# apirrone/Open_Duck_Playground

Measured on AMD Instinct MI355X. Metric: env-steps/sec open_duck_mini_v2 flat_terrain @8192 envs; 1/2/4/8-GPU scaling, higher is better.
Workload: dtype f32

## Files before the change

### open_duck_playground_amd/csrc/odk_engine.hip

```cpp
#include <hip/hip_runtime.h>
#include <stddef.h>

#include <cmath>
#include <cstdarg>
#include <cstdio>
#include <cstdlib>
#include <cstring>
#include <array>
#include <string>
#include <vector>

#include "../../include/odk.h"
#include "odk_kernels.h"

using namespace odk;

struct RecLay {
  int CMD, LAST, LAST2, LAST3, MT, AIR, PEAK, PUSH, AHIST, IMU, EPSTEPS, TRUNC, DONE, EPSUM, EPLEN, EPMET, KEY0, KEY1, CTR, STEP, PSTEP, PINT, IMI, LCON, NINFO;
};
constexpr RecLay rec_lay(int nu) {
  RecLay r{};
  r.CMD = 0; r.LAST = 7; r.LAST2 = r.LAST + nu; r.LAST3 = r.LAST2 + nu; r.MT = r.LAST3 + nu; r.AIR = r.MT + nu; r.PEAK = r.AIR + 2; r.PUSH = r.PEAK + 2;
  r.AHIST = r.PUSH + 2; r.IMU = r.AHIST + 3 * nu; r.EPSTEPS = r.IMU + 9; r.TRUNC = r.EPSTEPS + 1; r.DONE = r.TRUNC + 1; r.EPSUM = r.DONE + 1; r.EPLEN = r.EPSUM + 1;
  r.EPMET = r.EPLEN + 1; r.KEY0 = r.EPMET + ODK_NMETRIC; r.KEY1 = r.KEY0 + 1; r.CTR = r.KEY1 + 1; r.STEP = r.CTR + 1; r.PSTEP = r.STEP + 1; r.PINT = r.PSTEP + 1;
// ... 206 lines not shown

__device__ inline void sample_command(const EnvCfg& c, uint32_t k0, uint32_t k1, uint32_t ctr, uint32_t base, int k, float& out) {
  const float z = rng_uniform(k0, k1, ctr, base + 7);
  const float u = rng_uniform(k0, k1, ctr, base + k);
  out = (z < 0.1f) ? 0.0f : c.cmd_range[k][0] + u * (c.cmd_range[k][1] - c.cmd_range[k][0]);
}

template <int NDRAW>
__device__ __forceinline__ void draw_block(uint32_t k0, uint32_t k1, uint32_t ctr, float* NZ, int lane) {
  uint32_t a, b;
  threefry2x32(k0, k1, ctr, (uint32_t)(lane + 2), a, b);
  if (lane < NDRAW / 2) { NZ[2 * lane] = (float)(a >> 8) * (1.0f / 16777216.0f); NZ[2 * lane + 1] = (float)(b >> 8) * (1.0f / 16777216.0f); }
  ODK_SYNC();
}

template <class S, int G, int KIND>
__device__ __forceinline__ void build_obs_kind(float* L, const DevModel* m, const EnvCfg& c, const float* contact, const float* NZ,
                          int imitation_i, const float* phase, int lane) {
  using E = EnvL<S>;
  float* P = L + E::O_PRIV; float* INFO = L + E::O_INFO; const float* SENS = L + S::O_SENS; const float* SCR = L + S::O_SCR;
  const float* QPOS = L + S::O_QPOS; const float* QVEL = L + S::O_QVEL;
  const float lvl = c.noise_level;
  constexpr int NU = S::NU;
  constexpr RecLay RL = rec_lay(NU);
  constexpr int NOBS = obs_nobs(NU, false), DQV = draw_qvel(NU) - 4;
  const float con0 = contact[0], con1 = contact[1], ph0 = phase[0], ph1 = phase[1];
  const int adr_gyro = m->adr_gyro, adr_acc = m->adr_accelerometer, adr_lin = m->adr_local_linvel, adr_ang = m->adr_global_angvel;
  float ng = 0;
  if (lane < 3) ng = SCR[S::S_MISC + 10 + lane] + (2.0f * NZ[10 - 4 + lane] - 1.0f) * lvl * c.noise_gravity;
  float h0 = 0, h1 = 0;
  if (lane < 3) { h0 = INFO[RL.IMU + lane]; h1 = INFO[RL.IMU + 3 + lane]; }
  ODK_SYNC();
  if (lane < 3) { INFO[RL.IMU + lane] = ng; INFO[RL.IMU + 3 + lane] = h0; INFO[RL.IMU + 6 + lane] = h1; }
  constexpr bool standing = KIND != 0;
  constexpr int NP = obs_npriv(NU, standing);
#pragma unroll
  for (int it = 0; it < (NP + G - 1) / G; it++) {
    const int ks = lane + it * G;
    __builtin_assume(ks >= it * G && ks < it * G + G);
    if (ks >= NP) continue;
    const int k = !standing ? ks : (ks < 13 + 5 * NU ? ks : (ks < 15 + 5 * NU ? ks + NU : ks + NOBS - (15 + 5 * NU)));
    const int q = k - NOBS;
    const int uA = min(max(k - 13, 0), NU - 1), uV = min(max(k - 13 - NU, 0), NU - 1), uQ = min(max(q - 15, 0), NU - 1), uQV = min(max(q - 15 - NU, 0), NU - 1);
    const int tF = min(max(q - 18 - 3 * NU, 0), 5);
    const int A_bq = m->act_backlash_qposadr[uA], A_aq = m->act_qposadr[uA], V_ad = m->act_dofadr[uV];
    const float A_kc = m->key_ctrl[uA], A_ns = c.qpos_noise_scale[uA];
    const int Q_bq = m->act_backlash_qposadr[uQ], Q_aq = m->act_qposadr[uQ], QV_ad = m->act_dofadr[uQV], F_adr = m->adr_foot_linvel[tF >= 3 ? 1 : 0];
    const float Q_kc = m->key_ctrl[uQ];
    {
      const int k_lo = standing ? 0 : it * G, k_hi = standing ? NP + NOBS : it * G + G;
      auto hits = [&](int lo, int hi) { return k_lo < hi && k_hi > lo; };
      if (hits(13, 13 + NU)) asm volatile("" :: "v"(A_bq), "v"(A_aq), "v"(A_kc), "v"(A_ns));
      if (hits(13 + NU, 13 + 2 * NU)) asm volatile("" :: "v"(V_ad));
      if (hits(NOBS + 15, NOBS + 15 + NU)) asm volatile("" :: "v"(Q_bq), "v"(Q_aq), "v"(Q_kc));
      if (hits(NOBS + 15 + NU, NOBS + 15 + 2 * NU)) asm volatile("" :: "v"(QV_ad));
      if (hits(NOBS + 18 + 3 * NU, NOBS + 24 + 3 * NU)) asm volatile("" :: "v"(F_adr));
    }
    float v = 0;
    if (k < 3) v = SENS[adr_gyro + k] + (2.0f * NZ[k] - 1.0f) * lvl * c.noise_gyro;
    else if (k < 6) v = SENS[adr_acc + k - 3] + (2.0f * NZ[k] - 1.0f) * lvl * c.noise_accelerometer;
    else if (k < 13) v = INFO[RL.CMD + k - 6];
    else if (k < 13 + NU) {
      const int u = k - 13;
      const float ja = QPOS[A_aq] + (A_bq >= 0 ? QPOS[A_bq] : 0.0f);
      v = ja + (2.0f * NZ[13 - 4 + u] - 1.0f) * lvl * A_ns - A_kc;
    } else if (k < 13 + 2 * NU) {
      const int u = k - 13 - NU;
      v = (QVEL[V_ad] + (2.0f * NZ[DQV + u] - 1.0f) * lvl * c.noise_joint_vel) * c.dof_vel_scale;
    } else if (k < 13 + 3 * NU) v = INFO[RL.LAST + k - 13 - 2 * NU];
    else if (k < 13 + 4 * NU) v = INFO[RL.LAST2 + k - 13 - 3 * NU];
    else if (k < 13 + 5 * NU) v = INFO[RL.LAST3 + k - 13 - 4 * NU];
    else if (k < 13 + 6 * NU) v = INFO[RL.MT + k - 13 - 5 * NU];
    else if (k < 15 + 6 * NU) v = (k - 13 - 6 * NU) ? con1 : con0;
    else if (k < 17 + 6 * NU) v = (k - 15 - 6 * NU) ? ph1 : ph0;
    else {
      if (q < 3) v = SENS[adr_gyro + q];
      else if (q < 6) v = SENS[adr_acc + q - 3];
      else if (q < 9) v = SCR[S::S_MISC + 10 + q - 6];
      else if (q < 12) v = SENS[adr_lin + q - 9];
      else if (q < 15) v = SENS[adr_ang + q - 12];
      else if (q < 15 + NU) v = QPOS[Q_aq] + (Q_bq >= 0 ? QPOS[Q_bq] : 0.0f) - Q_kc;
      else if (q < 15 + 2 * NU) v = QVEL[QV_ad];
      else if (q == 15 + 2 * NU) v = QPOS[2];
      else if (q < 16 + 3 * NU) v = L[S::O_ACTF + q - 16 - 2 * NU];
      else if (q < 18 + 3 * NU) v = (q - 16 - 3 * NU) ? con1 : con0;
      else if (q < 24 + 3 * NU) { const int t = q - 18 - 3 * NU; v = SENS[F_adr + (t >= 3 ? t - 3 : t)]; }
      else if (q < 26 + 3 * NU) v = INFO[RL.AIR + q - 24 - 3 * NU];
      else if (q < 66 + 3 * NU) v = L[E::O_REF + q - 26 - 3 * NU];
      else if (q == 66 + 3 * NU) v = (float)imitation_i;
      else v = (q - 67 - 3 * NU) ? ph1 : ph0;
    }
    P[ks] = v;
  }
  ODK_SYNC();
}
template <class S, int G>
__device__ __forceinline__ void build_obs(float* L, const DevModel* m, const EnvCfg& c, const float* contact, const float* NZ,
                          int imitation_i, const float* phase, int lane) {
  if (c.kind == 0) build_obs_kind<S, G, 0>(L, m, c, contact, NZ, imitation_i, phase, lane);
  else build_obs_kind<S, G, 1>(L, m, c, contact, NZ, imitation_i, phase, lane);
}

__device__ __forceinline__ void foot_contact_flags(const float* CDIST, float* contact) {
  for (int f = 0; f < 2; f++) {
    float md = 1e4f;
    for (int k = 0; k < 4; k++) md = fminf(md, CDIST[4 * f + k]);
    contact[f] = md < 0 ? 1.0f : 0.0f;
  }
}

template <class S, int G>
__device__ __forceinline__ void write_outputs(const KArgs& a, const float* L, int env, float reward, float done, float trunc, const float* metrics, int lane) {
  using E = EnvL<S>;
  const float* P = L + E::O_PRIV;
  const int nobs = a.cfg.nobs, npriv = a.cfg.npriv;
// ... 121 lines not shown
    if (a.cmd) v = a.cmd[(size_t)e * a.cmd_stride + lane];
    INFO[RL.CMD + lane] = v;
  }
  ODK_SYNC();
  forward_env<S, G, HF>(L, RT, m, a.hfield, st, lane, 1);
  if (a.dbg_lds && live) dump_lds<S, G>(a.dbg_lds, L, env, lane);
  const float pint = c.push_interval_range[0] + rng_uniform(k0, kr, 0, 17 + NU) * (c.push_interval_range[1] - c.push_interval_range[0]);
  const int push_interval_steps = (int)rintf(pint / c.ctrl_dt);
  if (c.use_imitation) prm_eval<G>(&a.prm, a.prm_table, INFO[RL.CMD], INFO[RL.CMD + 1], INFO[RL.CMD + 2], 0, L + E::O_REF, lane);
  else for (int k = lane; k < 40; k += G) L[E::O_REF + k] = 0;
  ODK_SYNC();
  float contact[2];
  foot_contact_flags(L + S::O_CDIST, contact);
  const float phase[2] = {0, 0};
  draw_block<E::NDRAW>(k0, k1, 0u, L + E::O_NZ, lane);
  build_obs<S, G>(L, m, c, contact, L + E::O_NZ, 0, phase, lane);
  if (lane == 0) {
    INFO[RL.KEY0] = i2f((int)k0); INFO[RL.KEY1] = i2f((int)k1); INFO[RL.CTR] = i2f(1);
    INFO[RL.STEP] = i2f(0); INFO[RL.PSTEP] = i2f(0); INFO[RL.PINT] = i2f(push_interval_steps);
    INFO[RL.IMI] = i2f(0); INFO[RL.LCON] = i2f(0);
  }
  ODK_SYNC();
  if (live) {
    float* rc = a.recs + (size_t)env * R::SIZE;
    float* fs = a.first + (size_t)env * R::FSIZE;
    for (int i = lane; i < S::NQ; i += G) { rc[i] = L[S::O_QPOS + i]; fs[i] = L[S::O_QPOS + i]; }
    for (int i = lane; i < S::NV; i += G) {
      rc[S::NQ + i] = L[S::O_QVEL + i]; fs[S::NQ + i] = L[S::O_QVEL + i];
      rc[S::NQ + S::NV + i] = L[S::O_WARM + i]; fs[S::NQ + S::NV + i] = L[S::O_WARM + i];
    }
    for (int k = lane; k < R::NPRIV; k += G) {
      if (k < R::NOBS) fs[R::FOBS + k] = L[E::O_PRIV + k];
      fs[R::FOBS + R::NOBS + k] = L[E::O_PRIV + k];
    }
    for (int k = lane; k < RL.NINFO; k += G) rc[R::INFO + k] = INFO[k];
    float metrics[ODK_NMETRIC] = {0, 0, 0, 0, 0, 0, 0, 0};
    write_outputs<S, G>(a, L, env, 0.0f, 0.0f, 0.0f, metrics, lane);
    if (a.xmet && lane < ODK_NXTERM) a.xmet[(size_t)env * ODK_NXTERM + lane] = 0.0f;
  }
}

constexpr int STEP_WAVES = 2;
template <class S, int G, int HF>
__global__ void __launch_bounds__(64, STEP_WAVES) step_kernel(KArgs a) {
  extern __shared__ float lds[];
  using E = EnvL<S>; using R = Rec<S>;
  constexpr int NU = S::NU;
  constexpr RecLay RL = rec_lay(NU);
  const int slot = threadIdx.x / G, lane = threadIdx.x % G;
  const int env = blockIdx.x * (64 / G) + slot;
  const bool live = env < a.nenv;
  const int e = live ? env : a.nenv - 1;
  float* L = lds + slot * E::TOTAL;
#ifdef ODK_PROFILE
  const long long t_k0 = clock64();
#endif
  const int* RT = load_shared<S>(lds, 64 / G, a.m);
#ifdef ODK_POISON_LDS
  for (int k = lane; k < E::TOTAL; k += G) L[k] = __int_as_float(0x7fc00000);
// ... 83 lines not shown
  ODK_SYNC();
#ifdef ODK_PROFILE
  const long long t_k1 = clock64();
  if (lane == 0) L[S::O_SCR + S::S_PROF + 18] = (float)(t_k1 - t_k0);
#endif
  HotSt hot;
  if constexpr (HF == 0) load_hot<S, G>(hot, m, st, lane);
  for (int s = 0; s < a.n_substeps; s++) {
    const bool last = s == a.n_substeps - 1;
    size_t opaque0 = 0;
    asm volatile("" : "+s"(opaque0));
    const DevModel* ms = reinterpret_cast<const DevModel*>(reinterpret_cast<const char*>(m) + opaque0);
    int lane_s = lane;
    asm volatile("" : "+v"(lane_s));
    __builtin_assume(lane_s >= 0 && lane_s < 64);
    if constexpr (HF == 0) forward_env<S, G, HF, true>(L, RT, ms, a.hfield, st, lane_s, last ? 1 : 0, hot);
    else forward_env<S, G, HF>(L, RT, ms, a.hfield, st, lane_s, last ? 1 : 0);
    if (last && a.dbg_lds && live) dump_lds<S, G>(a.dbg_lds, L, env, lane);
    euler_env<S, G>(L, ms, st, lane_s);
  }
#ifdef ODK_PROFILE
  const long long t_k2 = clock64();
#endif
  size_t opaque1 = 0;
  asm volatile("" : "+s"(opaque1));
  const DevModel* mp = reinterpret_cast<const DevModel*>(reinterpret_cast<const char*>(m) + opaque1);
  const uint32_t k0e = (uint32_t)f2i(INFO[RL.KEY0]), k1e = (uint32_t)f2i(INFO[RL.KEY1]), ctre = (uint32_t)f2i(INFO[RL.CTR]);
  const int imi_e = f2i(INFO[RL.IMI]);
  const float phase_e[2] = {ACT[NU], ACT[NU + 1]};
  int step_e = f2i(INFO[RL.STEP]), push_step_e = f2i(INFO[RL.PSTEP]);
  float ep_steps_e = INFO[RL.EPSTEPS];
  const float prev_done_e = INFO[RL.DONE];
  for (int u = lane; u < NU; u += G) INFO[RL.MT + u] = CTRL[u];
  draw_block<E::NDRAW>(k0e, k1e, ctre, L + E::O_NZ, lane);
  if (lane < 40) L[E::O_REF + lane] = ref0;
  if (lane < 8) L[E::O_REF + 32 + lane] = ref1;
  ODK_SYNC();
  float contact[2];
  foot_contact_flags(L + S::O_CDIST, contact);
  float air[2], peak[2];
  for (int f = 0; f < 2; f++) {
    air[f] = INFO[RL.AIR + f] + dt;
    peak[f] = fmaxf(INFO[RL.PEAK + f], L[S::O_SCR + S::S_MISC + 8 + f]);
  }
  int fc_bits = 0;
  if (a.xt) {
    const int lc = f2i(INFO[RL.LCON]);
    for (int f = 0; f < 2; f++) fc_bits |= (INFO[RL.AIR + f] > 0.0f && (contact[f] != 0.0f || ((lc >> f) & 1))) ? 1 << f : 0;
  }
// ... 55 lines not shown
      const float lin_z = expf(-8.0f * (bv[2] - REF[36]) * (bv[2] - REF[36]));
      const float ang_xy = expf(-2.0f * ((bv[3] - REF[37]) * (bv[3] - REF[37]) + (bv[4] - REF[38]) * (bv[4] - REF[38]))) * 0.5f;
      const float ang_z = expf(-2.0f * (bv[5] - REF[39]) * (bv[5] - REF[39])) * 0.5f;
      float crew = 0;
      for (int f = 0; f < 2; f++) crew += (contact[f] == (REF[32 + f] > 0.5f ? 1.0f : 0.0f)) ? 1.0f : 0.0f;
      float r = lin_xy + lin_z + ang_xy + ang_z - t_jp * 15.0f - t_jv * 1.0e-3f + crew;
      r *= (cn > 0.01f) ? 1.0f : 0.0f;
      rew[6] = nan_to_num(r);
    }
  }
  float total = 0;
  for (int k = 0; k < 7; k++) { rew[k] *= c.reward_scales[k]; total += rew[k]; }
  if (a.xt) reward_library<S, G>(a, L, mp, contact, air, peak, fc_bits, done_env, total, env, live, lane);
  const float reward = fminf(fmaxf(total * dt, 0.0f), 10000.0f);
  const float* NZ = L + E::O_NZ;
  build_obs<S, G>(L, mp, c, contact, NZ, imi_e, phase_e, lane);
  step_e += 1; push_step_e += 1;
  float la = 0, lla = 0;
  for (int u = lane; u < NU; u += G) { la = INFO[RL.LAST + u]; lla = INFO[RL.LAST2 + u]; }
  ODK_SYNC();
  for (int u = lane; u < NU; u += G) { INFO[RL.LAST3 + u] = lla; INFO[RL.LAST2 + u] = la; INFO[RL.LAST + u] = ACT[u]; }
  if (step_e > 500 && lane < 7 && !a.cmd) {
    constexpr int DC = draw_cmd(NU) - 4;
    const float z = NZ[DC + 7], u = NZ[DC + lane];
    INFO[RL.CMD + lane] = (z < 0.1f) ? 0.0f : c.cmd_range[lane][0] + u * (c.cmd_range[lane][1] - c.cmd_range[lane][0]);
  }
  if (done_env || step_e > 500) step_e = 0;
  int lcon_new = 0;
  for (int f = 0; f < 2; f++) {
    if (contact[f] != 0.0f) { air[f] = 0; peak[f] = 0; lcon_new |= (1 << f); }
  }
// ... 21 lines not shown
    for (int k = lane; k < R::NPRIV; k += G) L[E::O_PRIV + k] = fs[R::FOBS + R::NOBS + k];
    if (a.cmd && lane >= 6 && lane < 13) L[E::O_PRIV + lane] = INFO[RL.CMD + lane - 6];
  }
  if (live) {
    int e_out = e;
    asm volatile("" : "+v"(e_out));
    float* rco = reinterpret_cast<float*>(reinterpret_cast<char*>(a.recs + (size_t)e_out * R::SIZE) + opaque1);
    for (int i = lane; i < S::NQ + 2 * S::NV; i += G) rco[i] = L[S::O_QPOS + i];
    for (int k = lane; k < RL.NINFO; k += G) rco[R::INFO + k] = INFO[k];
    write_outputs<S, G>(a, L, env, reward, done_f, trunc, metrics, lane);
  }
#ifdef ODK_PROFILE
  if (a.dbg_lds && live && lane == 0) a.dbg_lds[(size_t)env * S::TOTAL + S::O_SCR + S::S_PROF + 19] = (float)(clock64() - t_k2);
#endif
}

template <class S, int G, int HF>
__global__ void __launch_bounds__(64) physics_kernel(KArgs a) {
  extern __shared__ float lds[];
  using E = EnvL<S>; using R = Rec<S>;
  const int slot = threadIdx.x / G, lane = threadIdx.x % G;
  const int env = blockIdx.x * (64 / G) + slot;
  const bool live = env < a.nenv;
  const int e = live ? env : a.nenv - 1;
  float* L = lds + slot * E::TOTAL;
  const int* RT = load_shared<S>(lds, 64 / G, a.m);
#ifdef ODK_POISON_LDS
  for (int k = lane; k < E::TOTAL; k += G) L[k] = __int_as_float(0x7fc00000);
  ODK_SYNC();
#endif
// ... 402 lines not shown
      if (a > b) continue;
      if (ne >= maxe) return false;
      edge[ne][0] = a; edge[ne][1] = b; edge[ne][2] = f; edge[ne][3] = -1; ne++;
    }
  for (int f = 0; f < nf; f++)
    for (int i = 0; i < poly[f][0]; i++) {
      const int a = poly[f][1 + i], b = poly[f][1 + (i + 1) % poly[f][0]];
      if (a < b) continue;
      bool found = false;
      for (int k = 0; k < ne; k++) if (edge[k][0] == b && edge[k][1] == a) { edge[k][3] = f; found = true; }
      if (!found) return false;
    }
  for (int k = 0; k < ne; k++) if (edge[k][2] < 0 || edge[k][3] < 0) return false;
  *npoly = nf; *nedge = ne;
  return true;
}

extern "C" int odk_model_load(const void* blob, uint64_t len, odk_model** out) {
  if (!blob || !out || len < 16 || memcmp(blob, "ODKM", 4) != 0) return fail(ODK_ERR_INVALID, "odk_model_load: not an ODKM blob");
  Blob B{(const unsigned char*)blob, len};
  odk_model* mo = new odk_model();
  DevModel& m = mo->h;
  memset(&m, 0, sizeof(m));
  int one[1];
  B.I("nq", one, 1); m.nq = one[0]; B.I("nv", one, 1); m.nv = one[0]; B.I("nu", one, 1); m.nu = one[0];
  B.I("nbody", one, 1); m.nb = one[0]; B.I("njnt", one, 1); m.nj = one[0]; B.I("nsite", one, 1); m.nsite = one[0];
  if (!B.ok) { delete mo; return fail(ODK_ERR_INVALID, "odk_model_load: missing %s", B.missing.c_str()); }
  if (m.nq > MAXQ || m.nv > MAXV || m.nu > MAXU || m.nb > MAXB || m.nj > MAXJ || m.nsite > MAXSITE) { delete mo; return fail(ODK_ERR_UNSUPPORTED, "model too large"); }
  {
    RecHdr ch;
// ... 390 lines not shown
      m.dof_eqrow[d1] = r; if (d2 >= 0) m.dof_eqrow[d2] = r;
      m.neq++;
    }
  }
  if (mo->shape == 1 && !(m.paired && m.nvr == ShapeB::NVR && m.nMr == ShapeB::NMR && m.nHr == ShapeB::NHR)) {
    delete mo;
    return fail(ODK_ERR_UNSUPPORTED, "the 30-dof kernels expect backlash twins (same body, anchor and axis as their joint) over the 20-dof tree");
  }
  if (mo->shape != 1 && m.paired) { delete mo; return fail(ODK_ERR_UNSUPPORTED, "twin dofs in a model of the 20-dof shape"); }
  for (int lane = 0; lane < 64; lane++) {
    memset(&m.lane_st[lane], 0, sizeof(LaneSt));
#define X(i, S) if (mo->shape == i) compute_statics<S>(m.lane_st[lane], &m, lane);
    ODK_SHAPES(X)
#undef X
  }
  *out = mo;
  return ODK_OK;
}
extern "C" void odk_model_free(odk_model* m) { delete m; }
extern "C" int odk_model_dims(const odk_model* m, int* nq, int* nv, int* nu, int* nbody) {
  if (!m) return fail(ODK_ERR_INVALID, "null model");
  if (nq) *nq = m->h.nq; if (nv) *nv = m->h.nv; if (nu) *nu = m->h.nu; if (nbody) *nbody = m->h.nb;
  return ODK_OK;
}
extern "C" int odk_model_obs_sizes(const odk_model* m, int env_kind, int* nobs, int* npriv) {
  if (!m) return fail(ODK_ERR_INVALID, "null model");
  obs_sizes_nu(m->h.nu, env_kind, nobs, npriv);
  return ODK_OK;
}

// ... 139 lines not shown
  if (count != n) return fail(ODK_ERR_INVALID, "param %d expects %d values per env, got %d", param, n, count);
  for (int e = 0; e < b->nenv; e++) memcpy(&b->h_dr[(size_t)e * SIZE + off], v + (size_t)e * n, n * sizeof(float));
  HIPCHK(hipSetDevice(b->device));
  if (!b->d_dr) HIPCHK(hipMalloc(&b->d_dr, b->h_dr.size() * sizeof(float)));
  HIPCHK(hipMemcpy(b->d_dr, b->h_dr.data(), b->h_dr.size() * sizeof(float), hipMemcpyHostToDevice));
  return ODK_OK;
}

enum { K_RESET = 0, K_STEP = 1, K_PHYS = 2 };

template <class S, int G, int HF> static hipError_t launch_sg(int which, const KArgs& a, hipStream_t st) {
  const int per_block = 64 / G;
  const int grid = (a.nenv + per_block - 1) / per_block;
  const size_t lds = (size_t)EnvL<S>::wg_floats(per_block) * sizeof(float);
  if (which == K_RESET) hipLaunchKernelGGL((reset_kernel<S, G, HF>), dim3(grid), dim3(64), lds, st, a);
  else if (which == K_STEP) hipLaunchKernelGGL((step_kernel<S, G, HF>), dim3(grid), dim3(64), lds, st, a);
  else hipLaunchKernelGGL((physics_kernel<S, G, HF>), dim3(grid), dim3(64), lds, st, a);
  return hipGetLastError();
}
static hipError_t launch(odk_batch* b, int which, const KArgs& a, hipStream_t st) {
#if defined(ODK_DEV_C32)
  if (b->model.shape == 2 && b->G == 32) return launch_sg<ShapeC, 32, 0>(which, a, st);
  return hipErrorNotSupported;
#elif defined(ODK_DEV_D32)
  if (b->model.shape == 3 && b->G == 32) return launch_sg<ShapeD, 32, 0>(which, a, st);
  return hipErrorNotSupported;
#elif defined(ODK_DEV_B32)
  if (b->model.shape == 1 && b->model.h.floor_is_plane && b->G == 32) return launch_sg<ShapeB, 32, 0>(which, a, st);
  return hipErrorNotSupported;
#elif defined(ODK_DEV_A32)
  if (b->model.shape == 0 && b->G == 32) return launch_sg<ShapeA, 32, 0>(which, a, st);
// ... 378 lines not shown
  if (!strcmp(name, "HL")) return S::O_HL;
  if (!strcmp(name, "qfrc_smooth")) return S::O_QFS;
  if (!strcmp(name, "qacc_smooth")) return S::O_QAS;
  if (!strcmp(name, "x")) return S::O_X;
  if (!strcmp(name, "Ma")) return S::O_MA;
  if (!strcmp(name, "search")) return S::O_GRAD;
  if (!strcmp(name, "mv")) return S::O_MV;
  if (!strcmp(name, "efc_D")) return S::O_D;
  if (!strcmp(name, "efc_aref")) return S::O_AREF;
  if (!strcmp(name, "jar")) return S::O_JAR;
  if (!strcmp(name, "jv")) return S::O_JV;
  if (!strcmp(name, "W")) return S::O_W;
  if (!strcmp(name, "contact_dist")) return S::O_CDIST;
  if (!strcmp(name, "contact_r")) return S::O_CR;
  if (!strcmp(name, "scr")) return S::O_SCR;
  if (!strcmp(name, "sensordata")) return S::O_SENS;
  if (!strcmp(name, "actuator_force")) return S::O_ACTF;
  if (!strcmp(name, "qacc")) return S::O_QACC;
  return -1;
}
extern "C" int odk_lds_offset(const odk_batch* b, const char* name) {
  if (!b || !name) return -1;
#define X(i, S) if (b->model.shape == i) return lds_off<S>(name);
  ODK_SHAPES(X)
#undef X
  return -1;
}

extern "C" int odk_batch_get_state(odk_batch* b, float* qpos, float* qvel, float* warm) {
  if (!b) return fail(ODK_ERR_INVALID, "null");
// ... 44 lines not shown
```

### open_duck_playground_amd/csrc/odk_kernels.h

```cpp
#pragma once
#include <hip/hip_runtime.h>

#include "odk_model.h"

namespace odk {

#define ODK_SYNC() asm volatile("" ::: "memory")

constexpr float MINVAL_F = 1e-15f;
constexpr float PI_F = 3.14159265358979323846f;

struct EnvCfg {
  float ctrl_dt, action_scale, dof_vel_scale, max_motor_velocity;
  float noise_level, noise_gyro, noise_accelerometer, noise_gravity, noise_joint_vel;
  float qpos_noise_scale[16];
  float reward_scales[7];
  float tracking_sigma;
  float push_enable, push_interval_range[2], push_magnitude_range[2];
  float cmd_range[7][2];
  int use_imitation, use_motor_speed_limits, autoreset, episode_length, n_substeps;
  int kind, nobs, npriv;
  float reset_base_qvel;
};

// ... 1582 lines not shown
  const ConeEv e = cone_ev(Dn, Dm, mu, mur, x[0], x[1], x[2]);
  const float c1 = 0.5f * (Dn * x[0] * x[0] + Dt * (x[1] * x[1] + x[2] * x[2]));
  const float a1 = Dn * x[0] * v[0] + Dt * (x[1] * v[1] + x[2] * v[2]);
  const float b1 = Dn * v[0] * v[0] + Dt * (v[1] * v[1] + v[2] * v[2]);
  const float V0 = v[0] * mur, V1 = v[1] * mu, V2 = v[2] * mu;
  const float UV = e.U1 * V1 + e.U2 * V2, iT = __builtin_amdgcn_rcpf(e.zone == 2 ? e.T : 1.0f);
  const float cr = e.U1 * V2 - e.U2 * V1;
  const float T1 = UV * iT, T2 = cr * cr * iT * iT * iT;
  const float g1 = V0 - mur * T1;
  const float c2 = 0.5f * e.Dm * e.NmT * e.NmT, a2 = e.Dm * e.NmT * g1, b2 = e.Dm * (g1 * g1 - e.NmT * mur * T2);
  cost = e.zone == 0 ? 0.0f : (e.zone == 1 ? c1 : c2);
  d0 = e.zone == 0 ? 0.0f : (e.zone == 1 ? a1 : a2);
  d1 = e.zone == 0 ? 0.0f : (e.zone == 1 ? b1 : b2);
}

template <class S, int G, int HF, bool PRE = false>
__device__ __forceinline__ void forward_env(float* L, const int* RT, const DevModel* __restrict__ m, const float* __restrict__ hfield, const Statics<S, G>& st, int lane, int flags, const HotSt& hot = HotSt()) {
  const float* SH = reinterpret_cast<const float*>(RT);
  const float* CT = SH + S::SH_CT;
  constexpr int NV = S::NV, NB = S::NB, NR = S::NVR;
  using ST = Statics<S, G>;
  float* QPOS = L + S::O_QPOS; float* QVEL = L + S::O_QVEL; float* WARM = L + S::O_WARM; float* CTRL = L + S::O_CTRL;
  float* Q0 = L + S::O_Q0; float* MASS = L + S::O_MASS; float* ARM = L + S::O_ARM; float* FRL = L + S::O_FRL; float* KP = L + S::O_KP;
  float* XPOS = L + S::O_XPOS; float* XQUAT = L + S::O_XQUAT; float* CVEL = L + S::O_CVEL; float* CACC = L + S::O_CACC;
  float* CFRC = L + S::O_CFRC; float* CRB = L + S::O_CRB; float* SC = L + S::O_SC; float* CDOF = L + S::O_CDOF;
  float* BUF6 = L + S::O_BUF6; float* BUF6B = L + S::O_BUF6B; float* M = L + S::O_M; float* HL = L + S::O_HL;
  float* QFS = L + S::O_QFS; float* QAS = L + S::O_QAS; float* X = L + S::O_X; float* MA = L + S::O_MA; float* GRAD = L + S::O_GRAD;
  float* MV = L + S::O_MV; float* ED = L + S::O_D; float* AREF = L + S::O_AREF; float* JAR = L + S::O_JAR; float* JV = L + S::O_JV;
  float* W = L + S::O_W; float* CDIST = L + S::O_CDIST; float* CR = L + S::O_CR; float* SCR = L + S::O_SCR;
  float* SENS = L + S::O_SENS; float* ACTF = L + S::O_ACTF;
  const int nfl = m->nfl, nlim = m->nlim, r0c = nfl + nlim;
// ... 861 lines not shown
  { float r3[3] = {cost_s, gw, cost_w}; gsum_n<G, 3>(r3); cost_s = r3[0]; gauss_w = 0.5f * r3[1]; cost_w = r3[2] + gauss_w; }
  const bool use_warm = cost_w < cost_s;
  const float gauss = use_warm ? gauss_w : 0.0f;
  const float x = use_warm ? warm : qas;
  const float ma = use_warm ? ma_w : qfs;
  const float jar_fl = use_warm ? jar_fl_w : jar_fl_s, jar_lim = use_warm ? jar_lim_w : jar_lim_s;
  const float jar_eq = use_warm ? jar_eq_w : jar_eq_s;
  if constexpr (S::EQ) {
#pragma unroll
    for (int r = 0; r < EQP_ROWS; r++) pjar_s[r] = use_warm ? pjar_w[r] : pjar_s[r];
  }
#pragma unroll
  for (int t = 0; t < NCL; t++) {
    cjar[t] = use_warm ? cjv[t] : cjar[t];
    const int rc = lane + t * G;
    if (rc < S::NCROW) JAR[r0c + rc] = cjar[t];
  }
  ODK_PROF(10);
  float f_fl = 0, f_lim = 0;
  bool quad_fl = false;
  if (lane < nfl) { fl_cost(jar_fl, f_fl); quad_fl = (jar_fl > -fl_rf) && (jar_fl < fl_rf); }
  if (st.d_lim_on) quad_cost(lim_D, jar_lim, f_lim);
  if (lane < nfl) { MV[fs.dof] = f_fl; MA[fs.dof] = quad_fl ? fs.D : 0.0f; }
  {
    constexpr int NSLOT = (S::NCROW + G - 1) / G;
#pragma unroll
    for (int t = 0; t < NSLOT; t++) {
      if (t * G >= 32 && !any_ff) continue;
      const int rc = lane + t * G;
      const bool on = rc < S::NCROW;
      const int rcl = on ? rc : 0, r = r0c + rcl;
// ... 147 lines not shown
    if (both) {
      float cj[6];
#pragma unroll
      for (int k = 0; k < 6; k++) cj[k] = CDOF[k * NR + j];
      if (both & 1) {
#pragma unroll
        for (int k = 0; k < 6; k++) v += cj[k] * BUF6[k * NR + i];
      }
      if (both & 2) {
#pragma unroll
        for (int k = 0; k < 6; k++) v += cj[k] * BUF6B[k * NR + i];
      }
    }
    return v;
  };
  if (st.d_on) { MA[lane] = grad; GRAD[lane] = grad; }
  float rhs = grad;
  if constexpr (S::PAIRED) {
    ODK_SYNC();
    rhs = pair_rhs<S>(GRAD, ARM, JV, m, lane);
  }
  float search;
  if (!any_ffa) {
    {
      static_assert(G >= 21, "base x base entries must sit in the first pass");
      int ee[ST::NME]; float mm[ST::NME], hv[ST::NME];
#pragma unroll
      for (int t = 0; t < ST::NME; t++) { const int p = lane + t * G, pc = p < S::NMR ? p : 0; ee[t] = RT[pc]; mm[t] = M[pc]; }
#pragma unroll
      for (int t = 0; t < ST::NME; t++) {
        const int e = ee[t], i = e & 31, j = (e >> 5) & 31, both = (e >> 10) & (e >> 12) & 3, u = (e >> 16) & 31;
// ... 110 lines not shown
    if (np_rows > 0) {
      float s9[EQP_ROWS];
#pragma unroll
      for (int r = 0; r < EQP_ROWS; r++) s9[r] = st.d_on ? pj[r] * search : 0.0f;
      gsum_n<G, EQP_ROWS>(s9);
#pragma unroll
      for (int r = 0; r < EQP_ROWS; r++) if (r == lane && r < np_rows) { pr_D = EQW[S::EQP_D + r]; pr_jar = pjar_s[r]; pr_jv = s9[r]; }
    }
  }
#pragma unroll
  for (int t = 0; t < NCL; t++) {
    const int rc = lane + t * G;
    const bool on = rc < S::NCROW;
    cjv[t] = 0.0f;
    if (!(t * G >= 32 && !any_ff)) cjv[t] = (on && cD[t] > 0) ? contact_jx(rc, SCR + S::S_VF) : 0.0f;
    if (on) JV[r0c + rc] = cjv[t];
  }
  ODK_PROF(15);
  float ls_x[NCL][3], ls_v[NCL][3], ls_Dn[NCL], ls_Dt[NCL], ls_Dm[NCL], ls_mu[NCL], ls_mur[NCL], ls_on[NCL];
  if constexpr (S::ELL) {
    if (ell) {
#pragma unroll
      for (int t = 0; t < NCL; t++) {
        const int rc = lane + t * G;
        quad3(cjar[t], ls_x[t]); quad3(cjv[t], ls_v[t]);
        ls_Dn[t] = ODK_DPP(cD[t], 0x00, 0xF);
        ls_mu[t] = CT[(rc < S::NCROW ? rc : 0) >> 4];
        ls_mur[t] = ls_mu[t] * ell_mur; ls_Dt[t] = ls_Dn[t] * m->impratio; ls_Dm[t] = cone_dm(ls_Dn[t], ls_mur[t]);
        ls_on[t] = ((rc & 3) < 3 && rc < S::NCROW) ? 1.0f : 0.0f;
      }
    }
// ... 108 lines not shown
    if (s5) { hi_a = al[2]; hi_d0 = e0[2]; hi_d1 = e1[2]; }
    const bool s6 = (e0[0] > 0) && (hi_d0 > e0[0]);
    if (s6) { hi_a = al[0]; hi_d0 = e0[0]; hi_d1 = e1[0]; }
    swap = s1 || s2 || s3 || s4 || s5 || s6;
  }
  al[0] = lo_a; al[1] = hi_a; al[2] = 0.0f;
  ls_eval(Cost(), al, cs, e0, e1);
  const float lo_c = cs[0], hi_c = cs[1], p0_cost = cs[2];
  const bool improved = (lo_c < p0_cost) || (hi_c < p0_cost);
  const float alpha = improved ? (lo_c < hi_c ? lo_a : hi_a) : 0.0f;
  if (st.d_on) {
    const float xa = x + alpha * search;
    X[lane] = xa;
    WARM[lane] = xa;
  }
  if (lane == 0) { SCR[S::S_MISC + 13] = qg1; SCR[S::S_MISC + 14] = qg2; SCR[S::S_MISC + 15] = gauss; }
  if (lane == 0) { SCR[S::S_MISC + 4] = p0_d0; SCR[S::S_MISC + 5] = p0_d1; SCR[S::S_MISC + 6] = p0_cost; SCR[S::S_MISC + 7] = gtol; }
  if (lane == 0) { SCR[S::S_MISC + 1] = alpha; SCR[S::S_MISC + 2] = use_warm ? 1.0f : 0.0f; SCR[S::S_MISC + 3] = use_warm ? cost_w : cost_s; }
  ODK_SYNC();
  ODK_PROF(16);

  if (flags & 1) {
    if (lane < m->nsensor) {
      const int s = lane, site = m->sensor_site[s], b = m->site_body[site], type = m->sensor_type[s];
      float R[9], Rs[9], sp[3], dif[3], qb[4];
      for (int k = 0; k < 4; k++) qb[k] = XQUAT[k * NB + b];
      q2mat(R, qb);
      for (int i = 0; i < 3; i++)
        for (int j = 0; j < 3; j++) Rs[3 * i + j] = R[3 * i] * m->site_mat[site][j] + R[3 * i + 1] * m->site_mat[site][3 + j] + R[3 * i + 2] * m->site_mat[site][6 + j];
      for (int k = 0; k < 3; k++) {
        sp[k] = XPOS[k * NB + b] + R[3 * k] * m->site_pos[site][0] + R[3 * k + 1] * m->site_pos[site][1] + R[3 * k + 2] * m->site_pos[site][2];
        dif[k] = sp[k] - ref[k];
      }
// ... 84 lines not shown
```

### open_duck_playground_amd/csrc/odk_model.h

```cpp
#pragma once
#include <stdint.h>

namespace odk {

constexpr int EQ_MAX = 2;
constexpr int EQP_MAX = 2, EQP_ROWS = 9;
constexpr int MAXV = 32;
constexpr int MAXQ = 32;
constexpr int MAXB = 20;
constexpr int MAXJ = 26;
constexpr int MAXU = 16;
constexpr int MAXNZ = 512;
constexpr int MAXHV = 20;
constexpr int MAXHF = 40;
constexpr int MAXHE = 64;
constexpr int HULL_MAXV = 17;
constexpr int HULL_MAXF = 30;
constexpr int HULL_MAXE = 48;
static_assert(HULL_MAXV <= MAXHV && HULL_MAXF <= MAXHF && HULL_MAXE <= MAXHE && HULL_MAXF <= 32 && HULL_MAXE <= 48 && HULL_MAXV <= 17, "kernel hull regions");
constexpr int MAXCHAIN = 8;
constexpr int MAXSITE = 8;
constexpr int MAXSENS = 16;
constexpr int NCON = 12;
constexpr int NSENSD = 46;
// ... 4 lines not shown
  int body;
};

struct LaneSt {
  int j_qadr, j_dadr;
  int cs_pk;
  int ch_first, ch_len;
  int r_on, r_depth, r_Madr, r_ancmask, r_descmask, r_foot;
  int m_adr[16];
  int d_on, d_body;
  int d_act, d_flrow, d_limrow, d_foot;
  int d_qadr, d_lim_on;
  int d_tkind, d_red;
  float d_damping, d_lo, d_hi;
};

struct DevModel {
  BodySt body_st[2][64];
  LaneSt lane_st[64];
  int nq, nv, nu, nb, nj, nM, nH, nfl, nlim, nrow, nsite, nsensor;
  float dt, gravity[3], tolerance, ls_tolerance, impratio, meaninertia;
  int ls_iterations, iterations;
  int base_body, body_in_tree[MAXB], body_parent[MAXB], body_jntadr[MAXB], body_jntnum[MAXB];
  int max_level, body_level[MAXB], body_children[MAXB][4];
  int max_nonpath_level, body_pathmask[MAXB], body_is_path[MAXB], body_upmask[MAXB], body_path_head[MAXB];
  int np_count, np_body[4], np_nsrc[4], np_src[4][MAXB];
  int body_chain[MAXB][MAXCHAIN], body_chain_len[MAXB];
  int body_ancdof[MAXB][MAXV], body_nancdof[MAXB];
  int body_sub[MAXB][MAXB], body_nsub[MAXB];
  float body_pos[MAXB][3], body_quat[MAXB][4], body_ipos[MAXB][3], body_mass[MAXB], body_inertia[MAXB][6];
// ... 50 lines not shown
  float plane_pos[3], plane_n[3], plane_frame[9];
  int floor_is_plane;
  int hfield_nrow, hfield_ncol;
  float hfield_size[4], floor_mat[9];
  int hfield_filter;
  int site_body[MAXSITE], site_imu, site_feet[2];
  float site_pos[MAXSITE][3], site_mat[MAXSITE][9], site_quat[MAXSITE][4];
  int sensor_type[MAXSENS], sensor_site[MAXSENS], sensor_adr[MAXSENS];
  int adr_gyro, adr_local_linvel, adr_accelerometer, adr_upvector, adr_global_angvel, adr_foot_linvel[2];
  int eqp_cross;
  int neqp, eqp_nrow, eqp_type[EQP_MAX], eqp_b1[EQP_MAX], eqp_b2[EQP_MAX], eqp_row0[EQP_MAX], dof_eqp[MAXV];
  float eqp_a1[EQP_MAX][3], eqp_a2[EQP_MAX][3], eqp_relq[EQP_MAX][4], eqp_ts[EQP_MAX], eqp_imp[EQP_MAX][9], eqp_invw[EQP_MAX][2];
  int cone;
  int neq, eq_dof1[EQ_MAX], eq_dof2[EQ_MAX], eq_qadr1[EQ_MAX], eq_qadr2[EQ_MAX], eq_key[EQ_MAX], dof_eqrow[MAXV];
  float eq_poly[EQ_MAX][5], eq_imp[EQ_MAX][9], eq_invweight[EQ_MAX];
};

constexpr int PRISM_EDGE[9][4] = {{0, 1, 0, 2}, {1, 2, 0, 3}, {3, 5, 1, 4}, {0, 3, 2, 4}, {3, 4, 2, 1}, {1, 4, 3, 2}, {4, 5, 3, 1}, {2, 5, 4, 3}, {0, 2, 4, 0}};
constexpr int PRISM_POLY[5][5] = {{3, 0, 1, 2, 0}, {3, 3, 5, 4, 3}, {4, 0, 3, 4, 1}, {4, 1, 4, 5, 2}, {4, 2, 5, 3, 0}};

struct HfAssign { int v[625]; };
constexpr HfAssign make_hf_assign() {
  HfAssign T{};
  for (int idx = 0; idx < 625; idx++) {
    const int c[4] = {idx % 5, (idx / 5) % 5, (idx / 25) % 5, idx / 125};
    int asg[4] = {0, 0, 0, 0}, tgt[4] = {0, 1, 2, 3}, rnk[4] = {0, 0, 0, 0}, on[4] = {0, 0, 0, 0};
    for (int r = 0; r < 4; r++) if (c[r] > 0) { asg[r] = 1; on[r] = 1; }
    for (int r = 0; r < 4; r++) {
      if (on[r]) continue;
      int bt = -1, bl = 0;
// ... 19 lines not shown
```

Measured before the change: 19.85 million.

## Table-drive observation build, skip noise draws when noise off, split debug step kernel

Replaces the long per-element branch chain in build_obs with a host-precomputed gather table (source offsets, key ctrl, noise slot and flags) stored in the device model, and parks contact, phase and imitation values in scratch so every element becomes a uniform gather. The RNG draw block and the noise terms are skipped when noise_level is zero, unless some env in the wave is about to resample its command. Debug-only LDS writes in forward_env (JAR, JV, MA, solver diagnostics) are compiled out of the default step kernel, and a separate debug kernel variant is launched only when a dump buffer is requested. This trades divergent branching and redundant stores for table loads, and adds the risk that skipped draws or writes were needed somewhere.

Result: faster. 20.35 million (median of 6 runs) (+2.5%).

```diff
diff --git a/open_duck_playground_amd/csrc/odk_engine.hip b/open_duck_playground_amd/csrc/odk_engine.hip
--- a/open_duck_playground_amd/csrc/odk_engine.hip
+++ b/open_duck_playground_amd/csrc/odk_engine.hip
@@ -244,91 +244,54 @@
   ODK_SYNC();
 }
 
-template <class S, int G, int KIND>
-__device__ __forceinline__ void build_obs_kind(float* L, const DevModel* m, const EnvCfg& c, const float* contact, const float* NZ,
-                          int imitation_i, const float* phase, int lane) {
+template <class S, int G>
+__device__ __forceinline__ void build_obs(float* L, const DevModel* m, const EnvCfg& c, const float* contact, const float* NZ,
+                          int imitation_i, const float* phase, bool noisy, int lane) {
   using E = EnvL<S>;
-  float* P = L + E::O_PRIV; float* INFO = L + E::O_INFO; const float* SENS = L + S::O_SENS; const float* SCR = L + S::O_SCR;
-  const float* QPOS = L + S::O_QPOS; const float* QVEL = L + S::O_QVEL;
+  float* P = L + E::O_PRIV; float* INFO = L + E::O_INFO; float* SCR = L + S::O_SCR;
   const float lvl = c.noise_level;
   constexpr int NU = S::NU;
   constexpr RecLay RL = rec_lay(NU);
-  constexpr int NOBS = obs_nobs(NU, false), DQV = draw_qvel(NU) - 4;
-  const float con0 = contact[0], con1 = contact[1], ph0 = phase[0], ph1 = phase[1];
-  const int adr_gyro = m->adr_gyro, adr_acc = m->adr_accelerometer, adr_lin = m->adr_local_linvel, adr_ang = m->adr_global_angvel;
+  constexpr int NT = (obs_npriv(NU, false) + G - 1) / G;
+  static_assert(13 + NU <= G, "build_obs: the noisy joint angles (elements 13 .. 12 + nu) must lie in the first pass of G elements: nu <= G - 13 (see MAXU in odk_model.h)");
+  const ObsEnt* T = m->obs_tab[c.kind != 0 ? 1 : 0];
+  const int np = c.npriv;
+  ObsEnt ent[NT];
+#pragma unroll
+  for (int it = 0; it < NT; it++) { const int ks = lane + it * G; ent[it] = T[ks < np ? ks : 0]; }
   float ng = 0;
-  if (lane < 3) ng = SCR[S::S_MISC + 10 + lane] + (2.0f * NZ[10 - 4 + lane] - 1.0f) * lvl * c.noise_gravity;
+  if (lane < 3) { ng = SCR[S::S_MISC + 10 + lane]; if (noisy) ng = ng + (2.0f * NZ[10 - 4 + lane] - 1.0f) * lvl * c.noise_gravity; }
   float h0 = 0, h1 = 0;
   if (lane < 3) { h0 = INFO[RL.IMU + lane]; h1 = INFO[RL.IMU + 3 + lane]; }
+  if (lane == 0) {
+    SCR[S::S_MISC + OBS_PARK_CON] = contact[0]; SCR[S::S_MISC + OBS_PARK_CON + 1] = contact[1]; SCR[S::S_MISC + OBS_PARK_IMI] = (float)imitation_i;
+    SCR[S::S_MISC + OBS_PARK_PHASE] = phase[0]; SCR[S::S_MISC + OBS_PARK_PHASE + 1] = phase[1];
+  }
   ODK_SYNC();
   if (lane < 3) { INFO[RL.IMU + lane] = ng; INFO[RL.IMU + 3 + lane] = h0; INFO[RL.IMU + 6 + lane] = h1; }
-  constexpr bool standing = KIND != 0;
-  constexpr int NP = obs_npriv(NU, standing);
 #pragma unroll
-  for (int it = 0; it < (NP + G - 1) / G; it++) {
+  for (int it = 0; it < NT; it++) {
     const int ks = lane + it * G;
-    __builtin_assume(ks >= it * G && ks < it * G + G);
-    if (ks >= NP) continue;
-    const int k = !standing ? ks : (ks < 13 + 5 * NU ? ks : (ks < 15 + 5 * NU ? ks + NU : ks + NOBS - (15 + 5 * NU)));
-    const int q = k - NOBS;
-    const int uA = min(max(k - 13, 0), NU - 1), uV = min(max(k - 13 - NU, 0), NU - 1), uQ = min(max(q - 15, 0), NU - 1), uQV = min(max(q - 15 - NU, 0), NU - 1);
-    const int tF = min(max(q - 18 - 3 * NU, 0), 5);
-    const int A_bq = m->act_backlash_qposadr[uA], A_aq = m->act_qposadr[uA], V_ad = m->act_dofadr[uV];
-    const float A_kc = m->key_ctrl[uA], A_ns = c.qpos_noise_scale[uA];
-    const int Q_bq = m->act_backlash_qposadr[uQ], Q_aq = m->act_qposadr[uQ], QV_ad = m->act_dofadr[uQV], F_adr = m->adr_foot_linvel[tF >= 3 ? 1 : 0];
-    const float Q_kc = m->key_ctrl[uQ];
-    {
-      const int k_lo = standing ? 0 : it * G, k_hi = standing ? NP + NOBS : it * G + G;
-      auto hits = [&](int lo, int hi) { return k_lo < hi && k_hi > lo; };
-      if (hits(13, 13 + NU)) asm volatile("" :: "v"(A_bq), "v"(A_aq), "v"(A_kc), "v"(A_ns));
-      if (hits(13 + NU, 13 + 2 * NU)) asm volatile("" :: "v"(V_ad));
-      if (hits(NOBS + 15, NOBS + 15 + NU)) asm volatile("" :: "v"(Q_bq), "v"(Q_aq), "v"(Q_kc));
-      if (hits(NOBS + 15 + NU, NOBS + 15 + 2 * NU)) asm volatile("" :: "v"(QV_ad));
-      if (hits(NOBS + 18 + 3 * NU, NOBS + 24 + 3 * NU)) asm volatile("" :: "v"(F_adr));
-    }
-    float v = 0;
-    if (k < 3) v = SENS[adr_gyro + k] + (2.0f * NZ[k] - 1.0f) * lvl * c.noise_gyro;
-    else if (k < 6) v = SENS[adr_acc + k - 3] + (2.0f * NZ[k] - 1.0f) * lvl * c.noise_accelerometer;
-    else if (k < 13) v = INFO[RL.CMD + k - 6];
-    else if (k < 13 + NU) {
-      const int u = k - 13;
-      const float ja = QPOS[A_aq] + (A_bq >= 0 ? QPOS[A_bq] : 0.0f);
-      v = ja + (2.0f * NZ[13 - 4 + u] - 1.0f) * lvl * A_ns - A_kc;
-    } else if (k < 13 + 2 * NU) {
-      const int u = k - 13 - NU;
-      v = (QVEL[V_ad] + (2.0f * NZ[DQV + u] - 1.0f) * lvl * c.noise_joint_vel) * c.dof_vel_scale;
-    } else if (k < 13 + 3 * NU) v = INFO[RL.LAST + k - 13 - 2 * NU];
-    else if (k < 13 + 4 * NU) v = INFO[RL.LAST2 + k - 13 - 3 * NU];
-    else if (k < 13 + 5 * NU) v = INFO[RL.LAST3 + k - 13 - 4 * NU];
-    else if (k < 13 + 6 * NU) v = INFO[RL.MT + k - 13 - 5 * NU];
-    else if (k < 15 + 6 * NU) v = (k - 13 - 6 * NU) ? con1 : con0;
-    else if (k < 17 + 6 * NU) v = (k - 15 - 6 * NU) ? ph1 : ph0;
-    else {
-      if (q < 3) v = SENS[adr_gyro + q];
-      else if (q < 6) v = SENS[adr_acc + q - 3];
-      else if (q < 9) v = SCR[S::S_MISC + 10 + q - 6];
-      else if (q < 12) v = SENS[adr_lin + q - 9];
-      else if (q < 15) v = SENS[adr_ang + q - 12];
-      else if (q < 15 + NU) v = QPOS[Q_aq] + (Q_bq >= 0 ? QPOS[Q_bq] : 0.0f) - Q_kc;
-      else if (q < 15 + 2 * NU) v = QVEL[QV_ad];
-      else if (q == 15 + 2 * NU) v = QPOS[2];
-      else if (q < 16 + 3 * NU) v = L[S::O_ACTF + q - 16 - 2 * NU];
-      else if (q < 18 + 3 * NU) v = (q - 16 - 3 * NU) ? con1 : con0;
-      else if (q < 24 + 3 * NU) { const int t = q - 18 - 3 * NU; v = SENS[F_adr + (t >= 3 ? t - 3 : t)]; }
-      else if (q < 26 + 3 * NU) v = INFO[RL.AIR + q - 24 - 3 * NU];
-      else if (q < 66 + 3 * NU) v = L[E::O_REF + q - 26 - 3 * NU];
-      else if (q == 66 + 3 * NU) v = (float)imitation_i;
-      else v = (q - 67 - 3 * NU) ? ph1 : ph0;
-    }
+    if (ks >= np) continue;
+    const ObsEnt e = ent[it];
+    const float second = L[e.b >= 0 ? e.b : 0];
+    float v = L[e.a] + (e.b >= 0 ? second : ((e.fl & OBS_FL_PLUS0) ? 0.0f : -0.0f));
+    if (noisy) {
+      const int slot = e.fl & 255, nk = (e.fl >> 8) & 31;
+      float nq = 0.0f;
+      if (it == 0) {
+#pragma unroll
+        for (int u = 0; u < NU; u++) nq = nk - 3 == u ? c.qpos_noise_scale[u] : nq;
+      }
+      const float ns = nk == 0 ? c.noise_gyro : (nk == 1 ? c.noise_accelerometer : (nk == 2 ? c.noise_joint_vel : nq));
+      const float t = (2.0f * NZ[slot ? slot - 1 : 0] - 1.0f) * lvl;
+      v = v + (slot ? t : -0.0f) * (slot ? ns : 1.0f);
+    }
+    v = v - e.kc;
+    v = v * ((e.fl & OBS_FL_VEL) ? c.dof_vel_scale : 1.0f);
     P[ks] = v;
   }
   ODK_SYNC();
-}
-template <class S, int G>
-__device__ __forceinline__ void build_obs(float* L, const DevModel* m, const EnvCfg& c, const float* contact, const float* NZ,
-                          int imitation_i, const float* phase, int lane) {
-  if (c.kind == 0) build_obs_kind<S, G, 0>(L, m, c, contact, NZ, imitation_i, phase, lane);
-  else build_obs_kind<S, G, 1>(L, m, c, contact, NZ, imitation_i, phase, lane);
 }
 
 __device__ __forceinline__ void foot_contact_flags(const float* CDIST, float* contact) {
@@ -480,7 +443,7 @@
   foot_contact_flags(L + S::O_CDIST, contact);
   const float phase[2] = {0, 0};
   draw_block<E::NDRAW>(k0, k1, 0u, L + E::O_NZ, lane);
-  build_obs<S, G>(L, m, c, contact, L + E::O_NZ, 0, phase, lane);
+  build_obs<S, G>(L, m, c, contact, L + E::O_NZ, 0, phase, c.noise_level != 0.0f, lane);
   if (lane == 0) {
     INFO[RL.KEY0] = i2f((int)k0); INFO[RL.KEY1] = i2f((int)k1); INFO[RL.CTR] = i2f(1);
     INFO[RL.STEP] = i2f(0); INFO[RL.PSTEP] = i2f(0); INFO[RL.PINT] = i2f(push_interval_steps);
@@ -507,8 +470,13 @@
 }
 
 constexpr int STEP_WAVES = 2;
-template <class S, int G, int HF>
-__global__ void __launch_bounds__(64, STEP_WAVES) step_kernel(KArgs a) {
+#ifdef ODK_PROFILE
+constexpr bool STEP_DUMPS_ALWAYS = true;
+#else
+constexpr bool STEP_DUMPS_ALWAYS = false;
+#endif
+template <class S, int G, int HF, bool DBG>
+__device__ __forceinline__ void step_body(const KArgs& a) {
   extern __shared__ float lds[];
   using E = EnvL<S>; using R = Rec<S>;
   constexpr int NU = S::NU;
@@ -622,9 +590,11 @@
     int lane_s = lane;
     asm volatile("" : "+v"(lane_s));
     __builtin_assume(lane_s >= 0 && lane_s < 64);
-    if constexpr (HF == 0) forward_env<S, G, HF, true>(L, RT, ms, a.hfield, st, lane_s, last ? 1 : 0, hot);
-    else forward_env<S, G, HF>(L, RT, ms, a.hfield, st, lane_s, last ? 1 : 0);
-    if (last && a.dbg_lds && live) dump_lds<S, G>(a.dbg_lds, L, env, lane);
+    if constexpr (HF == 0) forward_env<S, G, HF, true, DBG>(L, RT, ms, a.hfield, st, lane_s, last ? 1 : 0, hot);
+    else forward_env<S, G, HF, false, DBG>(L, RT, ms, a.hfield, st, lane_s, last ? 1 : 0);
+    if constexpr (DBG || STEP_DUMPS_ALWAYS) {
+      if (last && a.dbg_lds && live) dump_lds<S, G>(a.dbg_lds, L, env, lane);
+    }
     euler_env<S, G>(L, ms, st, lane_s);
   }
 #ifdef ODK_PROFILE
@@ -640,7 +610,10 @@
   float ep_steps_e = INFO[RL.EPSTEPS];
   const float prev_done_e = INFO[RL.DONE];
   for (int u = lane; u < NU; u += G) INFO[RL.MT + u] = CTRL[u];
-  draw_block<E::NDRAW>(k0e, k1e, ctre, L + E::O_NZ, lane);
+  const bool noisy = c.noise_level != 0.0f;
+  const bool resamples = !a.cmd && step_e + 1 > 500;
+  if (noisy || __builtin_amdgcn_ballot_w64(resamples) != 0)
+    draw_block<E::NDRAW>(k0e, k1e, ctre, L + E::O_NZ, lane);
   if (lane < 40) L[E::O_REF + lane] = ref0;
   if (lane < 8) L[E::O_REF + 32 + lane] = ref1;
   ODK_SYNC();
@@ -726,7 +699,7 @@
   if (a.xt) reward_library<S, G>(a, L, mp, contact, air, peak, fc_bits, done_env, total, env, live, lane);
   const float reward = fminf(fmaxf(total * dt, 0.0f), 10000.0f);
   const float* NZ = L + E::O_NZ;
-  build_obs<S, G>(L, mp, c, contact, NZ, imi_e, phase_e, lane);
+  build_obs<S, G>(L, mp, c, contact, NZ, imi_e, phase_e, noisy, lane);
   step_e += 1; push_step_e += 1;
   float la = 0, lla = 0;
   for (int u = lane; u < NU; u += G) { la = INFO[RL.LAST + u]; lla = INFO[RL.LAST2 + u]; }
@@ -778,6 +751,11 @@
   if (a.dbg_lds && live && lane == 0) a.dbg_lds[(size_t)env * S::TOTAL + S::O_SCR + S::S_PROF + 19] = (float)(clock64() - t_k2);
 #endif
 }
+
+template <class S, int G, int HF>
+__global__ void __launch_bounds__(64, STEP_WAVES) step_kernel(KArgs a) { step_body<S, G, HF, false>(a); }
+template <class S, int G, int HF>
+__global__ void __launch_bounds__(64, STEP_WAVES) step_kernel_dbg(KArgs a) { step_body<S, G, HF, true>(a); }
 
 template <class S, int G, int HF>
 __global__ void __launch_bounds__(64) physics_kernel(KArgs a) {
@@ -1210,6 +1188,59 @@
   for (int k = 0; k < ne; k++) if (edge[k][2] < 0 || edge[k][3] < 0) return false;
   *npoly = nf; *nedge = ne;
   return true;
+}
+
+template <class S> static void build_obs_table(DevModel& m) {
+  using E = EnvL<S>;
+  constexpr int NU = S::NU;
+  constexpr RecLay RL = rec_lay(NU);
+  constexpr int NOBS = obs_nobs(NU, false);
+  static_assert(obs_npriv(NU, false) <= OBS_MAX && draw_count(NU) < 255 && 3 + NU <= 32, "ObsEnt");
+  const int MISC = S::O_SCR + S::S_MISC, INFO = E::O_INFO, SENS = S::O_SENS;
+  for (int kind = 0; kind < 2; kind++) {
+    const bool standing = kind != 0;
+    const int NP = obs_npriv(NU, standing);
+    for (int ks = 0; ks < OBS_MAX; ks++) {
+      ObsEnt e = {0, -1, 0.0f, 0};
+      if (ks < NP) {
+        const int k = !standing ? ks : (ks < 13 + 5 * NU ? ks : (ks < 15 + 5 * NU ? ks + NU : ks + NOBS - (15 + 5 * NU)));
+        const int q = k - NOBS;
+        auto noise = [&](int draw, int kind_) { e.fl |= (draw - 4 + 1) | kind_ << 8; };
+        auto joint = [&](int u) {
+          e.a = S::O_QPOS + m.act_qposadr[u];
+          if (m.act_backlash_qposadr[u] >= 0) e.b = S::O_QPOS + m.act_backlash_qposadr[u]; else e.fl |= OBS_FL_PLUS0;
+          e.kc = m.key_ctrl[u];
+        };
+        if (k < 3) { e.a = SENS + m.adr_gyro + k; noise(4 + k, 0); }
+        else if (k < 6) { e.a = SENS + m.adr_accelerometer + k - 3; noise(4 + k, 1); }
+        else if (k < 13) e.a = INFO + RL.CMD + k - 6;
+        else if (k < 13 + NU) { const int u = k - 13; joint(u); noise(13 + u, 3 + u); }
+        else if (k < 13 + 2 * NU) { const int u = k - 13 - NU; e.a = S::O_QVEL + m.act_dofadr[u]; noise(draw_qvel(NU) + u, 2); e.fl |= OBS_FL_VEL; }
+        else if (k < 13 + 3 * NU) e.a = INFO + RL.LAST + k - 13 - 2 * NU;
+        else if (k < 13 + 4 * NU) e.a = INFO + RL.LAST2 + k - 13 - 3 * NU;
+        else if (k < 13 + 5 * NU) e.a = INFO + RL.LAST3 + k - 13 - 4 * NU;
+        else if (k < 13 + 6 * NU) e.a = INFO + RL.MT + k - 13 - 5 * NU;
+        else if (k < 15 + 6 * NU) e.a = MISC + OBS_PARK_CON + k - 13 - 6 * NU;
+        else if (k < 17 + 6 * NU) e.a = MISC + OBS_PARK_PHASE + k - 15 - 6 * NU;
+        else if (q < 3) e.a = SENS + m.adr_gyro + q;
+        else if (q < 6) e.a = SENS + m.adr_accelerometer + q - 3;
+        else if (q < 9) e.a = MISC + 10 + q - 6;
+        else if (q < 12) e.a = SENS + m.adr_local_linvel + q - 9;
+        else if (q < 15) e.a = SENS + m.adr_global_angvel + q - 12;
+        else if (q < 15 + NU) joint(q - 15);
+        else if (q < 15 + 2 * NU) e.a = S::O_QVEL + m.act_dofadr[q - 15 - NU];
+        else if (q == 15 + 2 * NU) e.a = S::O_QPOS + 2;
+        else if (q < 16 + 3 * NU) e.a = S::O_ACTF + q - 16 - 2 * NU;
+        else if (q < 18 + 3 * NU) e.a = MISC + OBS_PARK_CON + q - 16 - 3 * NU;
+        else if (q < 24 + 3 * NU) { const int t = q - 18 - 3 * NU; e.a = SENS + m.adr_foot_linvel[t >= 3 ? 1 : 0] + (t >= 3 ? t - 3 : t); }
+        else if (q < 26 + 3 * NU) e.a = INFO + RL.AIR + q - 24 - 3 * NU;
+        else if (q < 66 + 3 * NU) e.a = E::O_REF + q - 26 - 3 * NU;
+        else if (q == 66 + 3 * NU) e.a = MISC + OBS_PARK_IMI;
+        else e.a = MISC + OBS_PARK_PHASE + q - 67 - 3 * NU;
+      }
+      m.obs_tab[kind][ks] = e;
+    }
+  }
 }
 
 extern "C" int odk_model_load(const void* blob, uint64_t len, odk_model** out) {
@@ -1630,6 +1661,9 @@
     ODK_SHAPES(X)
 #undef X
   }
+#define X(i, S) if (mo->shape == i) build_obs_table<S>(m);
+  ODK_SHAPES(X)
+#undef X
   *out = mo;
   return ODK_OK;
 }
@@ -1799,7 +1833,12 @@
   const int grid = (a.nenv + per_block - 1) / per_block;
   const size_t lds = (size_t)EnvL<S>::wg_floats(per_block) * sizeof(float);
   if (which == K_RESET) hipLaunchKernelGGL((reset_kernel<S, G, HF>), dim3(grid), dim3(64), lds, st, a);
-  else if (which == K_STEP) hipLaunchKernelGGL((step_kernel<S, G, HF>), dim3(grid), dim3(64), lds, st, a);
+  else if (which == K_STEP) {
+    if constexpr (!STEP_DUMPS_ALWAYS) {
+      if (a.dbg_lds) { hipLaunchKernelGGL((step_kernel_dbg<S, G, HF>), dim3(grid), dim3(64), lds, st, a); return hipGetLastError(); }
+    }
+    hipLaunchKernelGGL((step_kernel<S, G, HF>), dim3(grid), dim3(64), lds, st, a);
+  }
   else hipLaunchKernelGGL((physics_kernel<S, G, HF>), dim3(grid), dim3(64), lds, st, a);
   return hipGetLastError();
 }
@@ -2208,6 +2247,7 @@
   if (!strcmp(name, "contact_dist")) return S::O_CDIST;
   if (!strcmp(name, "contact_r")) return S::O_CR;
   if (!strcmp(name, "scr")) return S::O_SCR;
+  if (!strcmp(name, "misc")) return S::O_SCR + S::S_MISC;
   if (!strcmp(name, "sensordata")) return S::O_SENS;
   if (!strcmp(name, "actuator_force")) return S::O_ACTF;
   if (!strcmp(name, "qacc")) return S::O_QACC;
diff --git a/open_duck_playground_amd/csrc/odk_kernels.h b/open_duck_playground_amd/csrc/odk_kernels.h
--- a/open_duck_playground_amd/csrc/odk_kernels.h
+++ b/open_duck_playground_amd/csrc/odk_kernels.h
@@ -1620,7 +1620,7 @@
   d1 = e.zone == 0 ? 0.0f : (e.zone == 1 ? b1 : b2);
 }
 
-template <class S, int G, int HF, bool PRE = false>
+template <class S, int G, int HF, bool PRE = false, bool DBG = true>
 __device__ __forceinline__ void forward_env(float* L, const int* RT, const DevModel* __restrict__ m, const float* __restrict__ hfield, const Statics<S, G>& st, int lane, int flags, const HotSt& hot = HotSt()) {
   const float* SH = reinterpret_cast<const float*>(RT);
   const float* CT = SH + S::SH_CT;
@@ -2512,7 +2512,7 @@
   for (int t = 0; t < NCL; t++) {
     cjar[t] = use_warm ? cjv[t] : cjar[t];
     const int rc = lane + t * G;
-    if (rc < S::NCROW) JAR[r0c + rc] = cjar[t];
+    if constexpr (DBG) { if (rc < S::NCROW) JAR[r0c + rc] = cjar[t]; }
   }
   ODK_PROF(10);
   float f_fl = 0, f_lim = 0;
@@ -2690,7 +2690,7 @@
     }
     return v;
   };
-  if (st.d_on) { MA[lane] = grad; GRAD[lane] = grad; }
+  if (st.d_on) { if constexpr (DBG) MA[lane] = grad; GRAD[lane] = grad; }
   float rhs = grad;
   if constexpr (S::PAIRED) {
     ODK_SYNC();
@@ -2831,7 +2831,7 @@
     const bool on = rc < S::NCROW;
     cjv[t] = 0.0f;
     if (!(t * G >= 32 && !any_ff)) cjv[t] = (on && cD[t] > 0) ? contact_jx(rc, SCR + S::S_VF) : 0.0f;
-    if (on) JV[r0c + rc] = cjv[t];
+    if constexpr (DBG) { if (on) JV[r0c + rc] = cjv[t]; }
   }
   ODK_PROF(15);
   float ls_x[NCL][3], ls_v[NCL][3], ls_Dn[NCL], ls_Dt[NCL], ls_Dm[NCL], ls_mu[NCL], ls_mur[NCL], ls_on[NCL];
@@ -2970,9 +2970,11 @@
     X[lane] = xa;
     WARM[lane] = xa;
   }
-  if (lane == 0) { SCR[S::S_MISC + 13] = qg1; SCR[S::S_MISC + 14] = qg2; SCR[S::S_MISC + 15] = gauss; }
-  if (lane == 0) { SCR[S::S_MISC + 4] = p0_d0; SCR[S::S_MISC + 5] = p0_d1; SCR[S::S_MISC + 6] = p0_cost; SCR[S::S_MISC + 7] = gtol; }
-  if (lane == 0) { SCR[S::S_MISC + 1] = alpha; SCR[S::S_MISC + 2] = use_warm ? 1.0f : 0.0f; SCR[S::S_MISC + 3] = use_warm ? cost_w : cost_s; }
+  if constexpr (DBG) {
+    if (lane == 0) { SCR[S::S_MISC + 13] = qg1; SCR[S::S_MISC + 14] = qg2; SCR[S::S_MISC + 15] = gauss; }
+    if (lane == 0) { SCR[S::S_MISC + 4] = p0_d0; SCR[S::S_MISC + 5] = p0_d1; SCR[S::S_MISC + 6] = p0_cost; SCR[S::S_MISC + 7] = gtol; }
+    if (lane == 0) { SCR[S::S_MISC + 1] = alpha; SCR[S::S_MISC + 2] = use_warm ? 1.0f : 0.0f; SCR[S::S_MISC + 3] = use_warm ? cost_w : cost_s; }
+  }
   ODK_SYNC();
   ODK_PROF(16);
 
diff --git a/open_duck_playground_amd/csrc/odk_model.h b/open_duck_playground_amd/csrc/odk_model.h
--- a/open_duck_playground_amd/csrc/odk_model.h
+++ b/open_duck_playground_amd/csrc/odk_model.h
@@ -42,6 +42,11 @@
   int d_tkind, d_red;
   float d_damping, d_lo, d_hi;
 };
+
+struct ObsEnt { int a, b; float kc; int fl; };
+constexpr int OBS_FL_VEL = 1 << 13, OBS_FL_PLUS0 = 1 << 14;
+constexpr int OBS_MAX = 232;
+constexpr int OBS_PARK_CON = 1, OBS_PARK_IMI = 3, OBS_PARK_PHASE = 4;
 
 struct DevModel {
   BodySt body_st[2][64];
@@ -122,6 +127,7 @@
   int cone;
   int neq, eq_dof1[EQ_MAX], eq_dof2[EQ_MAX], eq_qadr1[EQ_MAX], eq_qadr2[EQ_MAX], eq_key[EQ_MAX], dof_eqrow[MAXV];
   float eq_poly[EQ_MAX][5], eq_imp[EQ_MAX][9], eq_invweight[EQ_MAX];
+  alignas(16) ObsEnt obs_tab[2][OBS_MAX];
 };
 
 constexpr int PRISM_EDGE[9][4] = {{0, 1, 0, 2}, {1, 2, 0, 3}, {3, 5, 1, 4}, {0, 3, 2, 4}, {3, 4, 2, 1}, {1, 4, 3, 2}, {4, 5, 3, 1}, {2, 5, 4, 3}, {0, 2, 4, 0}};
```
